# hsinnan75/Dart

Measured on AMD Instinct MI355X. Metric: M paired-end reads/sec (2x101 bp vs GRCh38-sized index), host to host; records bit-identical to CPU dart, higher is better.
Workload: dtype u64/u8 integer

## Files before the change

dart_amd/csrc/dg_pair.h:

```cpp
#pragma once
#include "../../include/dartgpu.h"
#include "dg_common.h"
#include "dg_chain.h"
#include "dg_report.h"

template <class R1, class R2>
__host__ __device__ inline void d_settle_pair(const DParams &pr, DRead &m1, R1 &p1, DRead &m2, R2 &p2)
{
    bool linked = p1.mate(m1.iBest) == m2.iBest;
    if (linked && !pr.multi_hit) return;
    if (!linked && m1.score > 0 && m2.score > 0) {
        int best_sum = 0;
        for (int i = 0; i < m1.CanNum; i++) {
            const int a = p1.aln(i), j = p1.mate(i);
            if (a <= 0 || j < 0) continue;
            const int b = p2.aln(j);
            if (b <= 0) continue;
            linked = true;
            if (a + b > best_sum) { best_sum = a + b; m1.iBest = i; m1.score = a; m2.iBest = j; m2.score = b; }
        }
    }
    if (linked) {
        for (int i = 0; i < m1.CanNum; i++) {
            const int j = p1.mate(i);
// ... 129 lines not shown
    for (int i = 1; i < n; i++) {
        const SKey x = key[i * S];
        int j = i;
        for (; j > 0 && key[(j - 1) * S] > x; j--) key[j * S] = key[(j - 1) * S];
        key[j * S] = x;
    }
}

#define SMALL_NW 8
__host__ __device__ inline bool d_small_nw_is_diagonal(uint64_t a8, uint64_t b8, int g)
{
    int sp[SMALL_NW], tp[SMALL_NW];
    uint8_t cb[SMALL_NW];
#pragma unroll
    for (int q = 0; q < SMALL_NW; q++) { sp[q] = -2 - (q + 1); tp[q] = -131072; cb[q] = q < g ? d_nt4((unsigned char)(b8 >> (8 * q))) : (uint8_t)7; }
    int diag0 = 0;
    bool leaves = false;
    for (int i = 1; i <= g; i++) {
        int left_s = -2 - i, left_r = -131072;
        const uint8_t ca = d_nt4((unsigned char)(a8 >> (8 * (i - 1))));
        int diag = diag0;
        diag0 = left_s;
#pragma unroll
        for (int q = 0; q < SMALL_NW; q++) {
            int x = left_r - 1, y = left_s - 3;
            const int r = x > y ? x : y;
            x = tp[q] - 1; y = sp[q] - 3;
            const int t = x > y ? x : y;
            const int sv = d_tr2(d_max3(diag + (ca == cb[q] ? 3 : -3), r, t));
            leaves = leaves || (q == i - 1 && (sv == r || sv == t));
            diag = sp[q];
            sp[q] = sv; tp[q] = t;
            left_s = sv; left_r = r;
        }
    }
    return !leaves;
}

struct ReadAscii {
    const unsigned char *p;
    __host__ __device__ __forceinline__ uint64_t get8(int i, int e) const { uint64_t v = 0; for (int t = 0; t < e; t++) v |= (uint64_t)p[i + t] << (8 * t); return v; }
    __host__ __device__ __forceinline__ int mismatches8(const DIndex &ix, int i, int e, int64_t g, bool &dash) const {
        const uint64_t ref = d_ref8(ix, g), a8 = get8(i, e), keep = e == 8 ? ~0ull : (1ull << (8 * e)) - 1ull, lo7 = 0x7F7F7F7F7F7F7F7Full, hi1 = 0x8080808080808080ull;
        const uint64_t x = (a8 ^ ref) & keep, y = (a8 ^ 0x2D2D2D2D2D2D2D2Dull) | ~keep;
        dash = dash || ((~(((y & lo7) + lo7) | y)) & hi1) != 0ull;
        return __builtin_popcountll((((x & lo7) + lo7) | x) & hi1);
    }
};
struct ReadWords {
    const uint32_t *w; int W2;
    __host__ __device__ __forceinline__ uint64_t get8(int i, int e) const {
        const int w0 = i >> 4, sh = (i & 15) << 1;
        const uint32_t chi = w[w0], clo = w0 + 1 < W2 ? w[w0 + 1] : 0u, mhi = w[W2 + w0], mlo = w0 + 1 < W2 ? w[W2 + w0 + 1] : 0xFFFFFFFFu;
        const uint32_t c16 = (sh ? (chi << sh) | (clo >> (32 - sh)) : chi) >> 16, m16 = (sh ? (mhi << sh) | (mlo >> (32 - sh)) : mhi) >> 16;
        uint64_t v = 0;
        for (int t = 0; t < e; t++) {
            const uint32_t c = (c16 >> (14 - 2 * t)) & 3u, m = (m16 >> (14 - 2 * t)) & 3u;
            v |= (uint64_t)(m ? 0x4Eu : ((0x54474341u >> (8u * c)) & 0xFFu)) << (8 * t);
        }
        return v;
    }
    __host__ __device__ __forceinline__ int mismatches8(const DIndex &ix, int i, int e, int64_t g, bool &dash) const {
        const int64_t L = ix.l_pac;
        uint32_t g16;
        if (g >= 0 && g + 8 <= L) g16 = (__builtin_bswap32(*(const uint32_a1 *)(ix.pac + (g >> 2))) << ((g & 3) << 1)) >> 16;
        else if (g >= L && g + 8 <= 2 * L) {
            const int64_t lo = 2 * L - 1 - g - 7;
            const uint32_t w = (__builtin_bswap32(*(const uint32_a1 *)(ix.pac + (lo >> 2))) << ((lo & 3) << 1)) >> 16;
            uint32_t r = ((w & 0x3333u) << 2) | ((w >> 2) & 0x3333u); r = ((r & 0x0F0Fu) << 4) | ((r >> 4) & 0x0F0Fu); r = ((r & 0x00FFu) << 8) | (r >> 8);
            g16 = ~r & 0xFFFFu;
        } else {
            const uint64_t ref = d_ref8(ix, g), a8 = get8(i, e), keep = e == 8 ? ~0ull : (1ull << (8 * e)) - 1ull, lo7 = 0x7F7F7F7F7F7F7F7Full, hi1 = 0x8080808080808080ull;
            const uint64_t x = (a8 ^ ref) & keep;
            return __builtin_popcountll((((x & lo7) + lo7) | x) & hi1);
        }
        const int w0 = i >> 4, sh = (i & 15) << 1;
        const uint32_t chi = w[w0], clo = w0 + 1 < W2 ? w[w0 + 1] : 0u, mhi = w[W2 + w0], mlo = w0 + 1 < W2 ? w[W2 + w0 + 1] : 0xFFFFFFFFu;
        const uint32_t c16 = (sh ? (chi << sh) | (clo >> (32 - sh)) : chi) >> 16, m16 = (sh ? (mhi << sh) | (mlo >> (32 - sh)) : mhi) >> 16;
        const uint32_t x = c16 ^ g16, keep = (0xFFFF0000u >> (2 * e)) & 0xFFFFu;
        return __builtin_popcount(((x | (x >> 1)) | m16) & 0x5555u & keep);
    }
};

template <int S, class RD>
__host__ __device__ inline bool d_unit_reports(const DIndex &ix, const LocTab &lt, const DParams &pr, bool first, const RD seq, int len,
                                               const SKey *key, uint32_t *cw, int nc, uint64_t *rw, int &n_slot, DRead &rd, uint32_t &n_cig, uint32_t &n_nw, uint32_t &n_cells)
{
    const int64_t L = ix.l_pac;
    rd.score = rd.sub_score = rd.mis_num = rd.mapq = rd.iBest = 0;
    rd.CanNum = nc > 0 ? nc : 1;
    for (int i = 0; i < nc; i++) {
        const uint32_t w = cw[i * S];
        if (cw_score(w) == 0) continue;
        const int n = cw_count(w), f = cw_first(w);
        const SKey k0 = key[f * S];
        const int64_t diag = sk_diag(k0);
        if (n > 1 && diag == -1) return false;
        SKey prev = k0;
        int aln = sk_rlen(k0), mis = 0;
        uint32_t calls = 0, cells = 0;
        for (int k = 1; k < n; k++) {
            const SKey cur = key[(f + k) * S];
            const int from = sk_rpos(prev) + sk_rlen(prev), g = sk_rpos(cur) - from;
            if (sk_diag(cur) != diag || g < 1) return false;
            const int64_t gp = sk_gpos(prev) + sk_rlen(prev);
            int nm = 0;
            bool dash = false;
            for (int q = 0; q < g; q += 8) nm += seq.mismatches8(ix, from + q, g - q < 8 ? g - q : 8, gp + q, dash);
            if (nm <= 2 && nm <= (int)(g * 0.2)) { aln += g - nm; mis += nm; }
            else if (g == 1 && !dash) { calls++; cells++; mis += 1; }
            else if (g <= SMALL_NW && !dash && d_small_nw_is_diagonal(seq.get8(from, g), d_ref8(ix, gp), g)) {
                calls++; cells += (uint32_t)(g * g); aln += g - nm; mis += nm;
            }
            else return false;
            aln += sk_rlen(cur);
            prev = cur;
        }
        const int64_t gPos = sk_gpos(k0), end_gPos = sk_gpos(prev) + sk_rlen(prev) - 1;
        if (n > 1 && ((gPos < L) != (end_gPos < L))) return false;
        const int head = sk_rpos(k0), span = sk_rpos(prev) + sk_rlen(prev) - head, tail = len - head - span;
        if (mis > pr.max_mismatch) aln = 0;
        if (n_slot >= PU_SLOTS) return false;
        const int slot = n_slot++;
        uint64_t w0 = 0;
        if (aln > 0) {
            const int lb = d_loc_lower_bound(lt, gPos);
            const int chr = lt.chr[lb];
            int64_t pos; int bdir;
            if (gPos < L) { bdir = first ? 1 : 0; pos = gPos + 1 - lt.off[chr]; }
            else { bdir = first ? 0 : 1; pos = lt.key[lb] - end_gPos + 1; }
            if (pos <= 0 || pos > 0xFFFFFFFFll || chr > 0xFFFF) return false;
            w0 = (uint64_t)pos | ((uint64_t)chr << 32) | ((uint64_t)aln << 48) | ((uint64_t)bdir << 60) | (1ull << 61);
            n_cig += 1u + (head > 0) + (tail > 0);
            if (aln > rd.score) { rd.iBest = i; rd.mis_num = mis; rd.sub_score = rd.score; rd.score = aln; }
            else if (aln == rd.score) rd.sub_score = rd.score;
        }
        rw[(2 * slot) * S] = w0;
        rw[(2 * slot + 1) * S] = (uint64_t)head | ((uint64_t)span << 12) | ((uint64_t)tail << 24) | ((uint64_t)mis << 48);
        cw[i * S] = (w & ~(15u << 27)) | ((uint32_t)slot << 27);
        n_nw += calls; n_cells += cells;
    }
    return true;
}

template <int S, class RD>
__host__ __device__ inline void d_unit_process_rd(const DIndex &ix, const LocTab &lt, const DParams &pr, bool paired, int n1, int n2, int len1, int len2,
                                               const RD seq1, const RD seq2, SKey *key, uint32_t *cw, uint64_t *rw,
                                               bool try_fast, UnitState &st)
{
    d_unit_sort<S>(key, n1);
    if (paired) d_unit_sort<S>(key + n1 * S, n2);
    int k = 0;
    st.nc[0] = d_cluster_seeds(lt, pr, len1, n1, [&](int i) { return key[i * S]; },
                               [&](int first, int count, int score, int64_t) { cw[(k++) * S] = cw_make(first, count, score); });
    st.nc[1] = 0;
    CandLds<S> a{key, cw, st.nc[0]}, b{key + n1 * S, cw + st.nc[0] * S, 0};
    if (paired) {
        st.nc[1] = b.cnt = d_cluster_seeds(lt, pr, len2, n2, [&](int i) { return key[(n1 + i) * S]; },
                                           [&](int first, int count, int score, int64_t) { cw[(k++) * S] = cw_make(first, count, score); });
    }
    PP_STAMP(st.pp, st.pt, 1);
    d_candidate_rules(paired, a, b);
    PP_STAMP(st.pp, st.pt, 2);
    st.fast = false; st.n_cig = 0; st.n_nw = st.n_cells = 0; st.flag0[0] = st.flag0[1] = 0;
    if (!try_fast) return;
    int n_slot = 0;
    uint32_t n_cig = 0, n_nw = 0, n_cells = 0;
    if (!d_unit_reports<S>(ix, lt, pr, true, seq1, len1, key, cw, st.nc[0], rw, n_slot, st.rd[0], n_cig, n_nw, n_cells)) return;
    if (paired && !d_unit_reports<S>(ix, lt, pr, false, seq2, len2, key + n1 * S, cw + st.nc[0] * S, st.nc[1], rw, n_slot, st.rd[1], n_cig, n_nw, n_cells)) return;
    PP_STAMP(st.pp, st.pt, 3);
    RepLds<S> p1{cw, rw, st.nc[0], 0}, p2{cw + st.nc[0] * S, rw, st.nc[1], 0};
    if (paired) {
        d_settle_pair(pr, st.rd[0], p1, st.rd[1], p2);
        d_flag_pair(st.rd[0], p1, st.rd[1], p2);
        d_mapq(st.rd[1], p2);
    } else d_flag_single(st.rd[0], p1);
    d_mapq(st.rd[0], p1);
    st.flag0[0] = p1.flag0; st.flag0[1] = p2.flag0;
    st.fast = true; st.n_cig = n_cig; st.n_nw = n_nw; st.n_cells = n_cells;
    PP_STAMP(st.pp, st.pt, 4);
}
template <int S>
__host__ __device__ inline void d_unit_process(const DIndex &ix, const DParams &pr, bool paired, int n1, int n2, int len1, int len2,
                                               const unsigned char *seq1, const unsigned char *seq2, SKey *key, uint32_t *cw, uint64_t *rw,
                                               bool try_fast, UnitState &st)
{
    d_unit_process_rd<S, ReadAscii>(ix, d_loc_tab(ix), pr, paired, n1, n2, len1, len2, ReadAscii{seq1}, ReadAscii{seq2}, key, cw, rw, try_fast, st);
}

struct CompactOut { dg_read_c *reads; dg_report_c *reports; uint32_t *cigar; unsigned int *bad; };
__host__ __device__ __forceinline__ bool d_compact_read(const dg_read_out &r, dg_read_c &o)
{
    o.score = (uint16_t)r.score; o.sub_score = (uint16_t)r.sub_score; o.mis_num = (uint16_t)r.mis_num; o.mapq = (uint8_t)r.mapq; o.n_sj = (uint8_t)r.n_sj;
    o.n_rep = (uint16_t)r.n_rep; o.best = (uint16_t)r.best;
    return !((uint32_t)r.score > 0xFFFFu || (uint32_t)r.sub_score > 0xFFFFu || (uint32_t)r.mis_num > 0xFFFFu || (uint32_t)r.mapq > 0xFFu || (uint32_t)r.n_sj > 0xFFu ||
             (uint32_t)r.n_rep > 0xFFFFu || (uint32_t)r.best > 0xFFFFu);
}
__host__ __device__ __forceinline__ bool d_compact_report(const dg_report_out &p, bool plain, bool slow, dg_report_c &q)
{
    q.pos = (int32_t)p.pos; q.aln_score = (uint16_t)p.aln_score; q.flag = (uint16_t)p.flag; q.paired_idx = (int16_t)p.paired_idx;
    q.chr = p.chr < 0 ? (uint16_t)0xFFFFu : (uint16_t)p.chr; q.sj_type = (int8_t)p.sj_type; q.bdir = (uint8_t)p.bdir; q.pad = slow ? 1u : 0u;
    q.n_cigar = plain ? (uint8_t)DG_CIGAR_FULL_MATCH : (uint8_t)p.n_cigar;
    return !(p.pos != (int64_t)(int32_t)p.pos || (uint32_t)p.aln_score > 0xFFFFu || (uint32_t)p.flag > 0xFFFFu || p.paired_idx > 32767 || p.paired_idx < -1 ||
             p.chr >= 0xFFFF || p.n_cigar > 254u || p.sj_type < -128 || p.sj_type > 127 || (uint32_t)p.bdir > 1u);
}

template <int S>
__host__ __device__ inline uint32_t d_unit_compact_ops(const DRead &rd, const RepLds<S> &p)
{
    uint32_t n = 0;
    for (int i = 0; i < rd.CanNum; i++) {
        const int s = p.slot(i);
        if (s == 15) continue;
        const uint64_t w0 = p.rw[(2 * s) * S], w1 = p.rw[(2 * s + 1) * S];
        if (!((w0 >> 61) & 1ull)) continue;
        const uint32_t head = (uint32_t)(w1 & 0xFFFu), tail = (uint32_t)((w1 >> 24) & 0xFFFu);
        n += (head || tail) ? 1u + (head > 0) + (tail > 0) : 0u;
    }
    return n;
}

template <int S>
__host__ __device__ inline uint32_t d_unit_emit_read(bool first, const DRead &rd, const RepLds<S> &p, uint32_t rep_off, uint32_t cig_off,
                                                     dg_read_out *rout_r, dg_report_out *reports, uint32_t *cigar, const CompactOut &co = CompactOut{nullptr, nullptr, nullptr, nullptr},
                                                     dg_read_c *rc_r = nullptr, uint32_t cigc_off = 0, bool full = true)
{
    dg_read_out o;
    o.score = rd.score; o.sub_score = rd.sub_score; o.mis_num = rd.mis_num; o.mapq = rd.mapq; o.n_rep = rd.CanNum; o.best = rd.iBest;
    o.rep_off = (int32_t)rep_off; o.sj_off = 0; o.n_sj = 0;
    if (full) *rout_r = o;
    bool fits = true;
    if (co.reads) { dg_read_c oc; fits = d_compact_read(o, oc); *rc_r = oc; }
    uint32_t used = 0, used_c = 0;
    for (int i = 0; i < rd.CanNum; i++) {
        dg_report_out rp;
        rp.aln_score = 0; rp.sj_type = -1; rp.flag = p.flag(i); rp.paired_idx = p.mate(i); rp.chr = -1; rp.bdir = 0; rp.pos = 0;
        rp.cigar_off = cig_off + used; rp.n_cigar = 0;
        const int s = p.slot(i);
        if (s != 15) {
            const uint64_t w0 = p.rw[(2 * s) * S], w1 = p.rw[(2 * s + 1) * S];
            if ((w0 >> 61) & 1ull) {
                rp.aln_score = (int32_t)((w0 >> 48) & 0xFFFu); rp.chr = (int32_t)((w0 >> 32) & 0xFFFFu); rp.bdir = (int32_t)((w0 >> 60) & 1u);
                rp.pos = (int64_t)(w0 & 0xFFFFFFFFull);
                const uint32_t head = (uint32_t)(w1 & 0xFFFu), span = (uint32_t)((w1 >> 12) & 0xFFFu), tail = (uint32_t)((w1 >> 24) & 0xFFFu);
                const bool rev = (rp.bdir != 0) != first;
                const uint32_t lead = rev ? tail : head, trail = rev ? head : tail;
                const uint32_t o_mid = CIG(span, OP_M), o_trail = CIG(trail, OP_S);
                const uint32_t a0 = lead ? CIG(lead, OP_S) : o_mid, a1 = lead ? o_mid : o_trail, a2 = o_trail;
                const uint32_t m = 1u + (lead ? 1u : 0u) + (trail ? 1u : 0u);
                if (full) { uint32_t *c = cigar + cig_off + used; c[0] = a0; if (m > 1) c[1] = a1; if (m > 2) c[2] = a2; }
                rp.n_cigar = m; used += m;
                if (co.reads && m > 1) { uint32_t *c = co.cigar + cigc_off + used_c; c[0] = a0; c[1] = a1; if (m > 2) c[2] = a2; used_c += m; }
            }
        }
        if (full) reports[rep_off + (uint32_t)i] = rp;
        if (co.reads) { dg_report_c q; fits = d_compact_report(rp, rp.n_cigar == 1u, false, q) && fits; co.reports[rep_off + (uint32_t)i] = q; }
    }
    if (co.reads && !fits) *co.bad = 1u;
    return used;
}

#include "dg_scan.h"

__device__ __forceinline__ uint32_t d_pac_touch(const DIndex &ix, SKey k)
{
    const int64_t L = ix.l_pac, g = sk_gpos(k) + sk_rlen(k);
    if (g >= 0 && g + 8 <= L) return *(const uint32_a1 *)(ix.pac + (g >> 2));
    if (g >= L && g + 8 <= 2 * L) return *(const uint32_a1 *)(ix.pac + ((2 * L - 1 - g - 7) >> 2));
    return 0u;
}

template <bool PACKED>
__global__ void __launch_bounds__(PU_THREADS)
k_pair(const DIndex ix, const DParams pr, int n_units, int paired, int try_fast, int write_all_sorted ,
       const unsigned char *__restrict__ seq, const uint32_t *__restrict__ seq_off, const uint32_t *__restrict__ enc, int W2, const uint16_t *__restrict__ rlen,
       const uint32_t *__restrict__ seed_off, SKey *__restrict__ seeds, DCand *__restrict__ cands, uint32_t *__restrict__ ncand,
       uint32_t *__restrict__ rep_off, uint32_t *__restrict__ slow_units,
       dg_read_out *__restrict__ rout, dg_report_out *__restrict__ reports, uint32_t *__restrict__ cigar,
       uint32_t cap_rep, uint32_t cap_cig, TileScan ts, DSizes *sizes, unsigned int *pool_top, unsigned long long *ctr, int *err, const CompactOut co)
{
    const unsigned long long t_wave0 = wall_clock64();
    __shared__ SKey s_key[PU_SEEDS * PU_THREADS];
    __shared__ uint32_t s_cw[PU_SEEDS * PU_THREADS];
    __shared__ uint64_t s_rw[2 * PU_SLOTS * PU_THREADS];
    __shared__ unsigned long long s_scan[20];
    __shared__ unsigned int s_tile;
    __shared__ int64_t s_lkey[PU_LOC_MAX]; __shared__ int64_t s_coff[PU_LOC_MAX / 2]; __shared__ int32_t s_lchr[PU_LOC_MAX];
    const bool tab_in_lds = 2 * ix.n_chr <= PU_LOC_MAX;
    if (tab_in_lds) {
        for (int i = threadIdx.x; i < 2 * ix.n_chr; i += PU_THREADS) { s_lkey[i] = ix.loc_key[i]; s_lchr[i] = ix.loc_chr[i]; }
        for (int i = threadIdx.x; i < ix.n_chr; i += PU_THREADS) s_coff[i] = ix.chr_off[i];
    }
    const LocTab lt = tab_in_lds ? LocTab{s_lkey, s_lchr, s_coff, 2 * ix.n_chr} : d_loc_tab(ix);
    bool leave = false;
    if (threadIdx.x == 0) { const int e0 = __hip_atomic_load(err, __ATOMIC_RELAXED, __HIP_MEMORY_SCOPE_AGENT); leave = e0 == DG_E_SEEDS || e0 == DG_E_SEEDQ || e0 == DG_E_SCAN; }
    const unsigned int tile = d_tile_ticket_unless(ts, &s_tile, leave);
    if (tile == SCAN_LEAVE) return;
    const int u = (int)(tile * PU_THREADS + threadIdx.x);
    const bool valid = u < n_units;
    SKey *key = s_key + threadIdx.x;
    uint32_t *cw = s_cw + threadIdx.x;
    uint64_t *rw = s_rw + threadIdx.x;
    UnitState st;
    st.fast = false; st.n_cig = 0; st.n_nw = st.n_cells = 0; st.nc[0] = st.nc[1] = 0; st.flag0[0] = st.flag0[1] = 0;
#ifdef DG_PAIR_PROF
    for (int i = 0; i < 10; i++) st.pp[i] = 0;
    st.pt = __builtin_amdgcn_s_memtime();
    const unsigned long long pp_t0 = st.pt;
#endif
    int r1 = 0, n1 = 0, n2 = 0, len1 = 0, len2 = 0;
    uint32_t b1 = 0;
    uint32_t pf = 0, pf2 = 0, pf3 = 0, pf4 = 0, pf5 = 0, pf6 = 0;
    bool heavy = false;
    if (valid) {
        r1 = paired ? 2 * u : u;
        len1 = rlen[r1]; len2 = paired ? rlen[r1 + 1] : 0;
        if (PACKED) { pf = enc[(size_t)r1 * 2 * W2 + (W2 >> 1)]; if (paired) pf2 = enc[(size_t)(r1 + 1) * 2 * W2 + (W2 >> 1)]; }
        b1 = seed_off[r1];
        const uint32_t e1 = seed_off[r1 + 1], e2 = paired ? seed_off[r1 + 2] : e1;
        n1 = (int)(e1 - b1); n2 = (int)(e2 - e1);
        heavy = n1 + n2 > PU_SEEDS;
        if (!heavy) {
            const SKey *src = seeds + b1;
            const int nt = n1 + n2;
            for (int i0 = 0; i0 < nt; i0 += 4) {
                const SKey k0 = src[i0], k1 = i0 + 1 < nt ? src[i0 + 1] : 0, k2 = i0 + 2 < nt ? src[i0 + 2] : 0, k3 = i0 + 3 < nt ? src[i0 + 3] : 0;
                key[i0 * PU_THREADS] = k0;
                if (i0 + 1 < nt) key[(i0 + 1) * PU_THREADS] = k1;
                if (i0 + 2 < nt) key[(i0 + 2) * PU_THREADS] = k2;
                if (i0 + 3 < nt) key[(i0 + 3) * PU_THREADS] = k3;
            }
#ifdef __HIP_DEVICE_COMPILE__
            __asm__ volatile("" ::: "memory");
#endif
            if (n1 > 1) { pf3 = d_pac_touch(ix, key[0]); if (n1 > 2) pf4 = d_pac_touch(ix, key[1 * PU_THREADS]); }
            if (n2 > 1) { pf5 = d_pac_touch(ix, key[n1 * PU_THREADS]); if (n2 > 2) pf6 = d_pac_touch(ix, key[(n1 + 1) * PU_THREADS]); }
            PP_STAMP(st.pp, st.pt, 0);
            if (PACKED) {
                const ReadWords a{enc + (size_t)r1 * 2 * W2, W2}, b{enc + (size_t)(r1 + (paired ? 1 : 0)) * 2 * W2, W2};
                d_unit_process_rd<PU_THREADS, ReadWords>(ix, lt, pr, paired != 0, n1, n2, len1, len2, a, b, key, cw, rw, try_fast != 0, st);
            } else d_unit_process_rd<PU_THREADS, ReadAscii>(ix, lt, pr, paired != 0, n1, n2, len1, len2, ReadAscii{seq + seq_off[r1]}, ReadAscii{seq + seq_off[r1 + (paired ? 1 : 0)]}, key, cw, rw, try_fast != 0, st);
        } else { st.nc[0] = (int)ncand[r1]; st.nc[1] = paired ? (int)ncand[r1 + 1] : 0; }
    }
    const uint32_t nrep1 = valid ? (uint32_t)(st.nc[0] > 0 ? st.nc[0] : 1) : 0u, nrep2 = (valid && paired) ? (uint32_t)(st.nc[1] > 0 ? st.nc[1] : 1) : 0u;
    Triple mine, tot;
    mine.x = nrep1 + nrep2; mine.y = (valid && !st.fast) ? 1u : 0u; mine.z = st.fast ? st.n_cig : 0u;
    uint32_t cc1 = 0;
    mine.w = 0;
    if (co.reads && st.fast) {
        RepLds<PU_THREADS> q1{cw, rw, st.nc[0], st.flag0[0]}, q2{cw + st.nc[0] * PU_THREADS, rw, st.nc[1], st.flag0[1]};
        cc1 = d_unit_compact_ops<PU_THREADS>(st.rd[0], q1);
        mine.w = cc1 + (paired ? d_unit_compact_ops<PU_THREADS>(st.rd[1], q2) : 0u);
    }
    PP_STAMP(st.pp, st.pt, 5);
    const Triple inb = d_block_exclusive(mine, tot, s_scan);
    PP_STAMP(st.pp, st.pt, 6);
    const Triple base = d_tile_exclusive(ts, tile, tot, s_scan + 16, err);
    PP_STAMP(st.pp, st.pt, 7);
    const uint32_t rep0 = base.x + inb.x, slow_at = base.y + inb.y;
    const uint64_t cig0 = base.z + inb.z;
    unsigned long long n_cands = 0, n_nw = 0, n_cells = 0;
    if (valid) {
        rep_off[r1] = rep0;
        if (paired) rep_off[r1 + 1] = rep0 + nrep1;
        if (!heavy) n_cands = (unsigned long long)(st.nc[0] + st.nc[1]);
        if (st.fast) {
            if ((uint64_t)rep0 + mine.x > cap_rep) atomicMax(err, DG_E_REPORTS);
            else if (cig0 + st.n_cig > cap_cig) atomicMax(err, DG_E_CIGFINAL);
            else {
                RepLds<PU_THREADS> p1{cw, rw, st.nc[0], st.flag0[0]}, p2{cw + st.nc[0] * PU_THREADS, rw, st.nc[1], st.flag0[1]};
                const uint32_t cigc0 = base.w + inb.w;
                const bool full = !(write_all_sorted & 2) || !co.reads;
                const uint32_t c1 = d_unit_emit_read<PU_THREADS>(true, st.rd[0], p1, rep0, (uint32_t)cig0, rout + r1, reports, cigar, co, co.reads ? co.reads + r1 : nullptr, cigc0, full);
                if (paired) d_unit_emit_read<PU_THREADS>(false, st.rd[1], p2, rep0 + nrep1, (uint32_t)cig0 + c1, rout + r1 + 1, reports, cigar, co, co.reads ? co.reads + r1 + 1 : nullptr, cigc0 + cc1, full);
                n_nw = st.n_nw; n_cells = st.n_cells;
            }
        } else {
            if (slow_at < (uint32_t)n_units) slow_units[slow_at] = (uint32_t)u;
            if ((uint64_t)rep0 + mine.x > cap_rep) atomicMax(err, DG_E_REPORTS);
        }
        if (!heavy && (!st.fast || (write_all_sorted & 1))) {
            const int nt = n1 + n2;
            for (int i = 0; i < nt; i++) seeds[b1 + i] = key[i * PU_THREADS];
            auto put_cands = [&](int first_cw, int first_key, uint32_t seg, int count, int r) {
                for (int i = 0; i < count; i++) {
                    const uint32_t w = cw[(first_cw + i) * PU_THREADS];
                    const int64_t d = sk_diag(key[(first_key + cw_first(w)) * PU_THREADS]);
                    DCand c = d_new_cand(seg + (uint32_t)cw_first(w), cw_count(w), cw_score(w), d < 0 ? 0 : d);
                    c.PairedIdx = cw_mate(w);
                    cands[seg + i] = c;
                }
                ncand[r] = (uint32_t)count;
            };
            put_cands(0, 0, b1, st.nc[0], r1);
            if (paired) put_cands(st.nc[0], n1, b1 + (uint32_t)n1, st.nc[1], r1 + 1);
        } else if (!heavy) { ncand[r1] = (uint32_t)st.nc[0]; if (paired) ncand[r1 + 1] = (uint32_t)st.nc[1]; }
    }
    if (tile == gridDim.x - 1 && threadIdx.x == 0) {
        sizes->total_rep = base.x + tot.x; sizes->n_slow_units = base.y + tot.y; sizes->cig_fast = (uint32_t)(base.z + tot.z);
        sizes->total_cig = sizes->cig_fast;
        sizes->pad[2] = base.w + tot.w;
        *pool_top = (base.x + tot.x) * CIG_SLOT;
    }
    PP_STAMP(st.pp, st.pt, 8);
#ifdef DG_PAIR_PROF
    if ((threadIdx.x & 63) == 0 && (tile % 61u) == 0u)
        printf("kpair tile %u wave %d: total %llu | load %llu sort+cluster %llu rules %llu reports %llu settle %llu rest %llu blockscan %llu lookback %llu emit %llu\n", tile, (int)(threadIdx.x >> 6),
               __builtin_amdgcn_s_memtime() - pp_t0, st.pp[0], st.pp[1], st.pp[2], st.pp[3], st.pp[4], st.pp[5], st.pp[6], st.pp[7], st.pp[8]);
#endif
    if (n_units < 0 && (pf ^ pf2 ^ pf3 ^ pf4 ^ pf5 ^ pf6) == 0x5A17C3E1u) atomicMax(err, DG_E_SCAN);
    d_wave_add(ctr + CTR_CANDS, n_cands);
    d_wave_add(ctr + CTR_NW, n_nw);
    d_wave_add(ctr + CTR_NWCELLS, n_cells);
    d_wave_resident(ctr, CTR_WT_PAIR, t_wave0);
}
```

Baseline: 1173.

## Distribute per-candidate report building and emission across wave lanes

Splits per-read report construction into independent per-candidate work items. Each lane handles its first candidate locally, and the remaining candidates are redistributed across the wave through a prefix scan and an owner search. Report emission and seed/candidate write-out are redistributed in the same way, so one lane no longer serialises all of its candidates. The goal is to reduce lane divergence and load imbalance from reads with many candidates. The cost is extra shuffles, wave-level LDS synchronisation, and calls/cells counters packed into the report word.

Result: no change. 1165 (-0.7%).

```diff
diff --git a/dart_amd/csrc/dg_pair.h b/dart_amd/csrc/dg_pair.h
--- a/dart_amd/csrc/dg_pair.h
+++ b/dart_amd/csrc/dg_pair.h
@@ -235,71 +235,96 @@
     }
 };
 
+#define PU_OUTSIDE (~0ull)
+#define PU_W1_SPENT ((0xFull << 60) | (0xFFFull << 36))
 template <int S, class RD>
-__host__ __device__ inline bool d_unit_reports(const DIndex &ix, const LocTab &lt, const DParams &pr, bool first, const RD seq, int len,
-                                               const SKey *key, uint32_t *cw, int nc, uint64_t *rw, int &n_slot, DRead &rd, uint32_t &n_cig, uint32_t &n_nw, uint32_t &n_cells)
+__host__ __device__ inline bool d_cand_report(const DIndex &ix, const LocTab &lt, const DParams &pr, bool first, const RD seq, int len,
+                                              const SKey *key, uint32_t w, uint64_t *rw, int slot)
 {
     const int64_t L = ix.l_pac;
+    rw[(2 * slot + 1) * S] = PU_OUTSIDE;
+    const int n = cw_count(w), f = cw_first(w);
+    const SKey k0 = key[f * S];
+    const int64_t diag = sk_diag(k0);
+    if (n > 1 && diag == -1) return false;
+    SKey prev = k0;
+    int aln = sk_rlen(k0), mis = 0;
+    uint32_t calls = 0, cells = 0;
+    for (int k = 1; k < n; k++) {
+        const SKey cur = key[(f + k) * S];
+        const int from = sk_rpos(prev) + sk_rlen(prev), g = sk_rpos(cur) - from;
+        if (sk_diag(cur) != diag || g < 1) return false;
+        const int64_t gp = sk_gpos(prev) + sk_rlen(prev);
+        int nm = 0;
+        bool dash = false;
+        for (int q = 0; q < g; q += 8) nm += seq.mismatches8(ix, from + q, g - q < 8 ? g - q : 8, gp + q, dash);
+        if (nm <= 2 && nm <= (int)(g * 0.2)) { aln += g - nm; mis += nm; }
+        else if (g == 1 && !dash) { calls++; cells++; mis += 1; }
+        else if (g <= SMALL_NW && !dash && d_small_nw_is_diagonal(seq.get8(from, g), d_ref8(ix, gp), g)) {
+            calls++; cells += (uint32_t)(g * g); aln += g - nm; mis += nm;
+        }
+        else return false;
+        aln += sk_rlen(cur);
+        prev = cur;
+    }
+    const int64_t gPos = sk_gpos(k0), end_gPos = sk_gpos(prev) + sk_rlen(prev) - 1;
+    if (n > 1 && ((gPos < L) != (end_gPos < L))) return false;
+    const int head = sk_rpos(k0), span = sk_rpos(prev) + sk_rlen(prev) - head, tail = len - head - span;
+    if (mis > pr.max_mismatch) aln = 0;
+    uint64_t w0 = 0;
+    if (aln > 0) {
+        const int lb = d_loc_lower_bound(lt, gPos);
+        const int chr = lt.chr[lb];
+        int64_t pos; int bdir;
+        if (gPos < L) { bdir = first ? 1 : 0; pos = gPos + 1 - lt.off[chr]; }
+        else { bdir = first ? 0 : 1; pos = lt.key[lb] - end_gPos + 1; }
+        if (pos <= 0 || pos > 0xFFFFFFFFll || chr > 0xFFFF) return false;
+        w0 = (uint64_t)pos | ((uint64_t)chr << 32) | ((uint64_t)aln << 48) | ((uint64_t)bdir << 60) | (1ull << 61);
+    }
+    if (calls > 15u || cells > 0xFFFu) return false;
+    rw[(2 * slot) * S] = w0;
+    rw[(2 * slot + 1) * S] = (uint64_t)head | ((uint64_t)span << 12) | ((uint64_t)tail << 24) | ((uint64_t)mis << 48) | ((uint64_t)cells << 36) | ((uint64_t)calls << 60);
+    return true;
+}
+
+template <int S>
+__host__ __device__ inline uint32_t d_unit_slots(uint32_t *cw, int nc)
+{
+    uint32_t live = 0, k = 0;
+    for (int i = 0; i < nc; i++) {
+        const uint32_t w = cw[i * S];
+        if (cw_score(w) == 0) continue;
+        cw[i * S] = (w & ~(15u << 27)) | ((k < 15u ? k : 15u) << 27);
+        live |= 1u << i; k++;
+    }
+    return live;
+}
+
+template <int S>
+__host__ __device__ inline bool d_mate_replay(const uint32_t *cw, int nc, uint64_t *rw, DRead &rd, uint32_t &n_cig, uint32_t &n_nw, uint32_t &n_cells)
+{
     rd.score = rd.sub_score = rd.mis_num = rd.mapq = rd.iBest = 0;
     rd.CanNum = nc > 0 ? nc : 1;
     for (int i = 0; i < nc; i++) {
         const uint32_t w = cw[i * S];
         if (cw_score(w) == 0) continue;
-        const int n = cw_count(w), f = cw_first(w);
-        const SKey k0 = key[f * S];
-        const int64_t diag = sk_diag(k0);
-        if (n > 1 && diag == -1) return false;
-        SKey prev = k0;
-        int aln = sk_rlen(k0), mis = 0;
-        uint32_t calls = 0, cells = 0;
-        for (int k = 1; k < n; k++) {
-            const SKey cur = key[(f + k) * S];
-            const int from = sk_rpos(prev) + sk_rlen(prev), g = sk_rpos(cur) - from;
-            if (sk_diag(cur) != diag || g < 1) return false;
-            const int64_t gp = sk_gpos(prev) + sk_rlen(prev);
-            int nm = 0;
-            bool dash = false;
-            for (int q = 0; q < g; q += 8) nm += seq.mismatches8(ix, from + q, g - q < 8 ? g - q : 8, gp + q, dash);
-            if (nm <= 2 && nm <= (int)(g * 0.2)) { aln += g - nm; mis += nm; }
-            else if (g == 1 && !dash) { calls++; cells++; mis += 1; }
-            else if (g <= SMALL_NW && !dash && d_small_nw_is_diagonal(seq.get8(from, g), d_ref8(ix, gp), g)) {
-                calls++; cells += (uint32_t)(g * g); aln += g - nm; mis += nm;
-            }
-            else return false;
-            aln += sk_rlen(cur);
-            prev = cur;
-        }
-        const int64_t gPos = sk_gpos(k0), end_gPos = sk_gpos(prev) + sk_rlen(prev) - 1;
-        if (n > 1 && ((gPos < L) != (end_gPos < L))) return false;
-        const int head = sk_rpos(k0), span = sk_rpos(prev) + sk_rlen(prev) - head, tail = len - head - span;
-        if (mis > pr.max_mismatch) aln = 0;
-        if (n_slot >= PU_SLOTS) return false;
-        const int slot = n_slot++;
-        uint64_t w0 = 0;
+        const int slot = cw_slot(w);
+        const uint64_t w0 = rw[(2 * slot) * S], w1 = rw[(2 * slot + 1) * S];
+        if (w1 == PU_OUTSIDE) return false;
+        n_nw += (uint32_t)(w1 >> 60); n_cells += (uint32_t)((w1 >> 36) & 0xFFFu);
+        rw[(2 * slot + 1) * S] = w1 & ~PU_W1_SPENT;
+        const int aln = (int)((w0 >> 48) & 0xFFFu);
         if (aln > 0) {
-            const int lb = d_loc_lower_bound(lt, gPos);
-            const int chr = lt.chr[lb];
-            int64_t pos; int bdir;
-            if (gPos < L) { bdir = first ? 1 : 0; pos = gPos + 1 - lt.off[chr]; }
-            else { bdir = first ? 0 : 1; pos = lt.key[lb] - end_gPos + 1; }
-            if (pos <= 0 || pos > 0xFFFFFFFFll || chr > 0xFFFF) return false;
-            w0 = (uint64_t)pos | ((uint64_t)chr << 32) | ((uint64_t)aln << 48) | ((uint64_t)bdir << 60) | (1ull << 61);
-            n_cig += 1u + (head > 0) + (tail > 0);
-            if (aln > rd.score) { rd.iBest = i; rd.mis_num = mis; rd.sub_score = rd.score; rd.score = aln; }
+            n_cig += 1u + ((w1 & 0xFFFu) != 0) + (((w1 >> 24) & 0xFFFu) != 0);
+            if (aln > rd.score) { rd.iBest = i; rd.mis_num = (int)((w1 >> 48) & 0xFFFu); rd.sub_score = rd.score; rd.score = aln; }
             else if (aln == rd.score) rd.sub_score = rd.score;
         }
-        rw[(2 * slot) * S] = w0;
-        rw[(2 * slot + 1) * S] = (uint64_t)head | ((uint64_t)span << 12) | ((uint64_t)tail << 24) | ((uint64_t)mis << 48);
-        cw[i * S] = (w & ~(15u << 27)) | ((uint32_t)slot << 27);
-        n_nw += calls; n_cells += cells;
     }
     return true;
 }
 
-template <int S, class RD>
-__host__ __device__ inline void d_unit_process_rd(const DIndex &ix, const LocTab &lt, const DParams &pr, bool paired, int n1, int n2, int len1, int len2,
-                                               const RD seq1, const RD seq2, SKey *key, uint32_t *cw, uint64_t *rw,
-                                               bool try_fast, UnitState &st)
+template <int S>
+__host__ __device__ inline void d_unit_candidates(const LocTab &lt, const DParams &pr, bool paired, int n1, int n2, int len1, int len2, SKey *key, uint32_t *cw, UnitState &st)
 {
     d_unit_sort<S>(key, n1);
     if (paired) d_unit_sort<S>(key + n1 * S, n2);
@@ -316,11 +341,14 @@
     d_candidate_rules(paired, a, b);
     PP_STAMP(st.pp, st.pt, 2);
     st.fast = false; st.n_cig = 0; st.n_nw = st.n_cells = 0; st.flag0[0] = st.flag0[1] = 0;
-    if (!try_fast) return;
-    int n_slot = 0;
+}
+
+template <int S>
+__host__ __device__ inline void d_unit_finish(const DParams &pr, bool paired, uint32_t *cw, uint64_t *rw, UnitState &st)
+{
     uint32_t n_cig = 0, n_nw = 0, n_cells = 0;
-    if (!d_unit_reports<S>(ix, lt, pr, true, seq1, len1, key, cw, st.nc[0], rw, n_slot, st.rd[0], n_cig, n_nw, n_cells)) return;
-    if (paired && !d_unit_reports<S>(ix, lt, pr, false, seq2, len2, key + n1 * S, cw + st.nc[0] * S, st.nc[1], rw, n_slot, st.rd[1], n_cig, n_nw, n_cells)) return;
+    if (!d_mate_replay<S>(cw, st.nc[0], rw, st.rd[0], n_cig, n_nw, n_cells)) return;
+    if (paired && !d_mate_replay<S>(cw + st.nc[0] * S, st.nc[1], rw, st.rd[1], n_cig, n_nw, n_cells)) return;
     PP_STAMP(st.pp, st.pt, 3);
     RepLds<S> p1{cw, rw, st.nc[0], 0}, p2{cw + st.nc[0] * S, rw, st.nc[1], 0};
     if (paired) {
@@ -333,6 +361,25 @@
     st.fast = true; st.n_cig = n_cig; st.n_nw = n_nw; st.n_cells = n_cells;
     PP_STAMP(st.pp, st.pt, 4);
 }
+
+template <int S, class RD>
+__host__ __device__ inline void d_unit_process_rd(const DIndex &ix, const LocTab &lt, const DParams &pr, bool paired, int n1, int n2, int len1, int len2,
+                                               const RD seq1, const RD seq2, SKey *key, uint32_t *cw, uint64_t *rw,
+                                               bool try_fast, UnitState &st)
+{
+    d_unit_candidates<S>(lt, pr, paired, n1, n2, len1, len2, key, cw, st);
+    if (!try_fast) return;
+    const uint32_t live = d_unit_slots<S>(cw, st.nc[0] + st.nc[1]);
+    if (__builtin_popcount(live) > PU_SLOTS) return;
+    for (int i = 0; i < st.nc[0] + st.nc[1]; i++) {
+        if (!((live >> i) & 1u)) continue;
+        const uint32_t w = cw[i * S];
+        const bool second = i >= st.nc[0];
+        if (!(second ? d_cand_report<S, RD>(ix, lt, pr, false, seq2, len2, key + n1 * S, w, rw, cw_slot(w))
+                     : d_cand_report<S, RD>(ix, lt, pr, true, seq1, len1, key, w, rw, cw_slot(w)))) return;
+    }
+    d_unit_finish<S>(pr, paired, cw, rw, st);
+}
 template <int S>
 __host__ __device__ inline void d_unit_process(const DIndex &ix, const DParams &pr, bool paired, int n1, int n2, int len1, int len2,
                                                const unsigned char *seq1, const unsigned char *seq2, SKey *key, uint32_t *cw, uint64_t *rw,
@@ -359,24 +406,60 @@
 }
 
 template <int S>
-__host__ __device__ inline uint32_t d_unit_compact_ops(const DRead &rd, const RepLds<S> &p)
+__host__ __device__ __forceinline__ uint32_t d_report_ops(const RepLds<S> &p, int i)
+{
+    const int s = p.slot(i);
+    if (s == 15) return 0u;
+    const uint64_t w0 = p.rw[(2 * s) * S], w1 = p.rw[(2 * s + 1) * S];
+    if (!((w0 >> 61) & 1ull)) return 0u;
+    const uint32_t head = (uint32_t)(w1 & 0xFFFu), tail = (uint32_t)((w1 >> 24) & 0xFFFu);
+    const uint32_t m = 1u + (head > 0) + (tail > 0);
+    return m | ((m > 1u ? m : 0u) << 16);
+}
+template <int S>
+__host__ __device__ inline uint32_t d_unit_ops(const DRead &rd, const RepLds<S> &p)
 {
     uint32_t n = 0;
-    for (int i = 0; i < rd.CanNum; i++) {
-        const int s = p.slot(i);
-        if (s == 15) continue;
+    for (int i = 0; i < rd.CanNum; i++) n += d_report_ops<S>(p, i);
+    return n;
+}
+template <int S>
+__host__ __device__ inline uint32_t d_unit_compact_ops(const DRead &rd, const RepLds<S> &p) { return d_unit_ops<S>(rd, p) >> 16; }
+
+template <int S>
+__host__ __device__ __forceinline__ uint32_t d_emit_report(bool first, const RepLds<S> &p, int i, uint32_t rep_at, uint32_t cig_at, uint32_t cigc_at,
+                                                           dg_report_out *reports, uint32_t *cigar, const CompactOut &co, bool full, bool &fits, uint32_t &ops_c)
+{
+    dg_report_out rp;
+    rp.aln_score = 0; rp.sj_type = -1; rp.flag = p.flag(i); rp.paired_idx = p.mate(i); rp.chr = -1; rp.bdir = 0; rp.pos = 0;
+    rp.cigar_off = cig_at; rp.n_cigar = 0;
+    ops_c = 0;
+    const int s = p.slot(i);
+    if (s != 15) {
         const uint64_t w0 = p.rw[(2 * s) * S], w1 = p.rw[(2 * s + 1) * S];
-        if (!((w0 >> 61) & 1ull)) continue;
-        const uint32_t head = (uint32_t)(w1 & 0xFFFu), tail = (uint32_t)((w1 >> 24) & 0xFFFu);
-        n += (head || tail) ? 1u + (head > 0) + (tail > 0) : 0u;
-    }
-    return n;
+        if ((w0 >> 61) & 1ull) {
+            rp.aln_score = (int32_t)((w0 >> 48) & 0xFFFu); rp.chr = (int32_t)((w0 >> 32) & 0xFFFFu); rp.bdir = (int32_t)((w0 >> 60) & 1u);
+            rp.pos = (int64_t)(w0 & 0xFFFFFFFFull);
+            const uint32_t head = (uint32_t)(w1 & 0xFFFu), span = (uint32_t)((w1 >> 12) & 0xFFFu), tail = (uint32_t)((w1 >> 24) & 0xFFFu);
+            const bool rev = (rp.bdir != 0) != first;
+            const uint32_t lead = rev ? tail : head, trail = rev ? head : tail;
+            const uint32_t o_mid = CIG(span, OP_M), o_trail = CIG(trail, OP_S);
+            const uint32_t a0 = lead ? CIG(lead, OP_S) : o_mid, a1 = lead ? o_mid : o_trail, a2 = o_trail;
+            const uint32_t m = 1u + (lead ? 1u : 0u) + (trail ? 1u : 0u);
+            if (full) { uint32_t *c = cigar + cig_at; c[0] = a0; if (m > 1) c[1] = a1; if (m > 2) c[2] = a2; }
+            rp.n_cigar = m;
+            if (co.reads && m > 1) { uint32_t *c = co.cigar + cigc_at; c[0] = a0; c[1] = a1; if (m > 2) c[2] = a2; ops_c = m; }
+        }
+    }
+    if (full) reports[rep_at] = rp;
+    if (co.reads) { dg_report_c q; fits = d_compact_report(rp, rp.n_cigar == 1u, false, q) && fits; co.reports[rep_at] = q; }
+    return rp.n_cigar;
 }
 
 template <int S>
 __host__ __device__ inline uint32_t d_unit_emit_read(bool first, const DRead &rd, const RepLds<S> &p, uint32_t rep_off, uint32_t cig_off,
                                                      dg_read_out *rout_r, dg_report_out *reports, uint32_t *cigar, const CompactOut &co = CompactOut{nullptr, nullptr, nullptr, nullptr},
-                                                     dg_read_c *rc_r = nullptr, uint32_t cigc_off = 0, bool full = true)
+                                                     dg_read_c *rc_r = nullptr, uint32_t cigc_off = 0, bool full = true, bool only_first = false)
 {
     dg_read_out o;
     o.score = rd.score; o.sub_score = rd.sub_score; o.mis_num = rd.mis_num; o.mapq = rd.mapq; o.n_rep = rd.CanNum; o.best = rd.iBest;
@@ -385,32 +468,78 @@
     bool fits = true;
     if (co.reads) { dg_read_c oc; fits = d_compact_read(o, oc); *rc_r = oc; }
     uint32_t used = 0, used_c = 0;
-    for (int i = 0; i < rd.CanNum; i++) {
-        dg_report_out rp;
-        rp.aln_score = 0; rp.sj_type = -1; rp.flag = p.flag(i); rp.paired_idx = p.mate(i); rp.chr = -1; rp.bdir = 0; rp.pos = 0;
-        rp.cigar_off = cig_off + used; rp.n_cigar = 0;
-        const int s = p.slot(i);
-        if (s != 15) {
-            const uint64_t w0 = p.rw[(2 * s) * S], w1 = p.rw[(2 * s + 1) * S];
-            if ((w0 >> 61) & 1ull) {
-                rp.aln_score = (int32_t)((w0 >> 48) & 0xFFFu); rp.chr = (int32_t)((w0 >> 32) & 0xFFFFu); rp.bdir = (int32_t)((w0 >> 60) & 1u);
-                rp.pos = (int64_t)(w0 & 0xFFFFFFFFull);
-                const uint32_t head = (uint32_t)(w1 & 0xFFFu), span = (uint32_t)((w1 >> 12) & 0xFFFu), tail = (uint32_t)((w1 >> 24) & 0xFFFu);
-                const bool rev = (rp.bdir != 0) != first;
-                const uint32_t lead = rev ? tail : head, trail = rev ? head : tail;
-                const uint32_t o_mid = CIG(span, OP_M), o_trail = CIG(trail, OP_S);
-                const uint32_t a0 = lead ? CIG(lead, OP_S) : o_mid, a1 = lead ? o_mid : o_trail, a2 = o_trail;
-                const uint32_t m = 1u + (lead ? 1u : 0u) + (trail ? 1u : 0u);
-                if (full) { uint32_t *c = cigar + cig_off + used; c[0] = a0; if (m > 1) c[1] = a1; if (m > 2) c[2] = a2; }
-                rp.n_cigar = m; used += m;
-                if (co.reads && m > 1) { uint32_t *c = co.cigar + cigc_off + used_c; c[0] = a0; c[1] = a1; if (m > 2) c[2] = a2; used_c += m; }
-            }
-        }
-        if (full) reports[rep_off + (uint32_t)i] = rp;
-        if (co.reads) { dg_report_c q; fits = d_compact_report(rp, rp.n_cigar == 1u, false, q) && fits; co.reports[rep_off + (uint32_t)i] = q; }
+    const int n = only_first ? 1 : rd.CanNum;
+    for (int i = 0; i < n; i++) {
+        uint32_t ops_c;
+        used += d_emit_report<S>(first, p, i, rep_off + (uint32_t)i, cig_off + used, cigc_off + used_c, reports, cigar, co, full, fits, ops_c);
+        used_c += ops_c;
     }
     if (co.reads && !fits) *co.bad = 1u;
     return used;
+}
+
+__device__ __forceinline__ void d_wave_lds_sync()
+{
+#ifdef __HIP_DEVICE_COMPILE__
+    __builtin_amdgcn_fence(__ATOMIC_RELEASE, "wavefront");
+    __builtin_amdgcn_wave_barrier();
+    __builtin_amdgcn_fence(__ATOMIC_ACQUIRE, "wavefront");
+#endif
+}
+__device__ __forceinline__ uint32_t d_wave_inclusive(uint32_t v)
+{
+    const int lane = (int)(threadIdx.x & 63u);
+    for (int o = 1; o < 64; o <<= 1) { const uint32_t up = (uint32_t)__shfl_up((int)v, o, 64); if (lane >= o) v += up; }
+    return v;
+}
+__device__ __forceinline__ int d_wave_owner(uint32_t incl, uint32_t j)
+{
+    int own = 0;
+    for (int step = 32; step; step >>= 1) { const uint32_t v = (uint32_t)__shfl((int)incl, own + step - 1, 64); if (v <= j) own += step; }
+    return own & 63;
+}
+
+template <int S>
+__host__ __device__ inline void d_item_emit_report(bool first, const RepLds<S> &p, int i, uint32_t rep_first, uint32_t cig_first, uint32_t cigc_first,
+                                                   dg_report_out *reports, uint32_t *cigar, const CompactOut &co, bool full)
+{
+    uint32_t before = 0;
+    for (int j = 0; j < i; j++) before += d_report_ops<S>(p, j);
+    bool fits = true;
+    uint32_t ops_c;
+    d_emit_report<S>(first, p, i, rep_first + (uint32_t)i, cig_first + (before & 0xFFFFu), cigc_first + (before >> 16), reports, cigar, co, full, fits, ops_c);
+    if (co.reads && !fits) *co.bad = 1u;
+}
+__host__ __device__ __forceinline__ int pu_extra_reports(int nc) { return nc > 1 ? nc - 1 : 0; }
+__host__ __device__ __forceinline__ void pu_item_report(int nc0, int k, int &mate, int &i)
+{
+    const int e0 = pu_extra_reports(nc0);
+    mate = k >= e0 ? 1 : 0;
+    i = (mate ? k - e0 : k) + 1;
+}
+__device__ __forceinline__ void d_wave_emit_reports(bool emit, int nc0, int nc1, uint32_t rep0, uint32_t cig0, uint32_t cigc0, uint32_t ops1, uint32_t *s_cw, uint64_t *s_rw,
+                                                    dg_report_out *reports, uint32_t *cigar, const CompactOut &co, bool full)
+{
+    const int lane = (int)(threadIdx.x & 63u), wave0 = (int)(threadIdx.x & ~63u);
+    uint32_t incl = emit ? (uint32_t)(pu_extra_reports(nc0) + pu_extra_reports(nc1)) : 0u;
+    if (__ballot(incl != 0u) == 0ull) return;
+    incl = d_wave_inclusive(incl);
+    const uint32_t total = (uint32_t)__shfl((int)incl, 63, 64), pk = (uint32_t)nc0 | ((uint32_t)nc1 << 5);
+    for (uint32_t base = 0; base < total; base += 64u) {
+        const uint32_t j = base + (uint32_t)lane;
+        const int own = d_wave_owner(incl, j);
+        const uint32_t o_incl = (uint32_t)__shfl((int)incl, own, 64), o_pk = (uint32_t)__shfl((int)pk, own, 64), o_rep0 = (uint32_t)__shfl((int)rep0, own, 64),
+                       o_cig0 = (uint32_t)__shfl((int)cig0, own, 64), o_cigc0 = (uint32_t)__shfl((int)cigc0, own, 64), o_ops1 = (uint32_t)__shfl((int)ops1, own, 64);
+        if (j < total) {
+            const int c0 = (int)(o_pk & 31u), c1 = (int)(o_pk >> 5);
+            int mate, i;
+            pu_item_report(c0, (int)(j - (o_incl - (uint32_t)(pu_extra_reports(c0) + pu_extra_reports(c1)))), mate, i);
+            const int t = wave0 + own;
+            const RepLds<PU_THREADS> p{s_cw + t + (mate ? c0 * PU_THREADS : 0), s_rw + t, mate ? c1 : c0, 0};
+            d_item_emit_report<PU_THREADS>(mate == 0, p, i, o_rep0 + (mate ? (uint32_t)(c0 > 0 ? c0 : 1) : 0u), o_cig0 + (mate ? (o_ops1 & 0xFFFFu) : 0u), o_cigc0 + (mate ? (o_ops1 >> 16) : 0u),
+                                           reports, cigar, co, full);
+        }
+    }
 }
 
 #include "dg_scan.h"
@@ -421,6 +550,100 @@
     if (g >= 0 && g + 8 <= L) return *(const uint32_a1 *)(ix.pac + (g >> 2));
     if (g >= L && g + 8 <= 2 * L) return *(const uint32_a1 *)(ix.pac + ((2 * L - 1 - g - 7) >> 2));
     return 0u;
+}
+
+template <int S>
+__host__ __device__ __forceinline__ void d_item_put_cand(const SKey *key, const uint32_t *cw, int n1, int nc0, uint32_t b1, int i, DCand *__restrict__ cands)
+{
+    const bool second = i >= nc0;
+    const int first_key = second ? n1 : 0;
+    const uint32_t seg = b1 + (uint32_t)first_key, w = cw[i * S];
+    const int64_t d = sk_diag(key[(first_key + cw_first(w)) * S]);
+    DCand c = d_new_cand(seg + (uint32_t)cw_first(w), cw_count(w), cw_score(w), d < 0 ? 0 : d);
+    c.PairedIdx = cw_mate(w);
+    cands[seg + (uint32_t)(i - (second ? nc0 : 0))] = c;
+}
+#define PU_ITEM_GROUP 16
+__host__ __device__ __forceinline__ uint32_t pu_counts_pack(int n1, int n2, int nc0, int nc1) { return (uint32_t)n1 | ((uint32_t)n2 << 5) | ((uint32_t)nc0 << 10) | ((uint32_t)nc1 << 15); }
+template <int S>
+__host__ __device__ __forceinline__ void d_item_write_out(const SKey *key, const uint32_t *cw, uint32_t pk, uint32_t b1, int i, SKey *__restrict__ seeds, DCand *__restrict__ cands)
+{
+    const int n1 = (int)(pk & 31u), n2 = (int)((pk >> 5) & 31u), nc0 = (int)((pk >> 10) & 31u), nc1 = (int)((pk >> 15) & 31u);
+    if (i < n1 + n2) seeds[b1 + (uint32_t)i] = key[i * S];
+    if (i < nc0 + nc1) d_item_put_cand<S>(key, cw, n1, nc0, b1, i, cands);
+}
+__host__ __device__ __forceinline__ int pu_take_owner(unsigned long long &m)
+{
+    const int o = m ? (int)__builtin_ctzll(m) : -1;
+    m &= m - 1ull;
+    return o;
+}
+static_assert(PU_ITEM_GROUP == PU_SEEDS && 64 / PU_ITEM_GROUP == 4 && PU_SEEDS < 32, "a group of lanes covers a unit's seeds, four groups a wave; the counts fit five bits");
+__device__ __forceinline__ void d_wave_write_out(bool wr, uint32_t pk, uint32_t b1, const SKey *s_key, const uint32_t *s_cw, SKey *__restrict__ seeds, DCand *__restrict__ cands)
+{
+    unsigned long long m = __ballot(wr);
+    const int lane = (int)(threadIdx.x & 63u), wave0 = (int)(threadIdx.x & ~63u), grp = lane / PU_ITEM_GROUP, i = lane % PU_ITEM_GROUP;
+    while (m) {
+        const int o0 = pu_take_owner(m), o1 = pu_take_owner(m), o2 = pu_take_owner(m), o3 = pu_take_owner(m);
+        const int o = grp == 0 ? o0 : (grp == 1 ? o1 : (grp == 2 ? o2 : o3));
+        const uint32_t opk = (uint32_t)__shfl((int)pk, o < 0 ? lane : o, 64), ob1 = (uint32_t)__shfl((int)b1, o < 0 ? lane : o, 64);
+        if (o >= 0) d_item_write_out<PU_THREADS>(s_key + wave0 + o, s_cw + wave0 + o, opk, ob1, i, seeds, cands);
+    }
+}
+
+__host__ __device__ __forceinline__ uint32_t pu_report_items(uint32_t live, int nc0) { return live & ~1u & ~(1u << nc0); }
+__host__ __device__ __forceinline__ int pu_kth_bit(uint32_t x, int k) { for (int t = 0; t < k; t++) x &= x - 1u; return __builtin_ctz(x); }
+template <bool PACKED> struct PuRead;
+template <> struct PuRead<true> {
+    __device__ static __forceinline__ ReadWords of(const unsigned char *, const uint32_t *, const uint32_t *enc, int W2, int r) { return ReadWords{enc + (size_t)r * 2 * W2, W2}; }
+};
+template <> struct PuRead<false> {
+    __device__ static __forceinline__ ReadAscii of(const unsigned char *seq, const uint32_t *seq_off, const uint32_t *, int, int r) { return ReadAscii{seq + seq_off[r]}; }
+};
+template <bool PACKED>
+__device__ __forceinline__ void d_wave_reports(const DIndex &ix, const LocTab &lt, const DParams &pr, bool go, int paired, int u, int n1, int len1, int len2,
+                                               const unsigned char *seq, const uint32_t *seq_off, const uint32_t *enc, int W2, const uint16_t *rlen,
+                                               SKey *s_key, uint32_t *s_cw, uint64_t *s_rw, UnitState &st)
+{
+    typedef PuRead<PACKED> R;
+    const int lane = (int)(threadIdx.x & 63u), wave0 = (int)(threadIdx.x & ~63u);
+    SKey *key = s_key + threadIdx.x; uint32_t *cw = s_cw + threadIdx.x; uint64_t *rw = s_rw + threadIdx.x;
+    const int r1 = paired ? 2 * u : u;
+    uint32_t live = 0;
+    bool ok = false;
+    if (go) {
+        live = d_unit_slots<PU_THREADS>(cw, st.nc[0] + st.nc[1]);
+        ok = __builtin_popcount(live) <= PU_SLOTS;
+#pragma unroll 1
+        for (int m = 0; m < 2; m++) {
+            const int c = m ? st.nc[0] : 0;
+            if (!ok || !((live >> c) & 1u)) continue;
+            const uint32_t w = cw[c * PU_THREADS];
+            ok = d_cand_report<PU_THREADS>(ix, lt, pr, m == 0, R::of(seq, seq_off, enc, W2, r1 + m), m ? len2 : len1, key + (m ? n1 * PU_THREADS : 0), w, rw, cw_slot(w));
+        }
+    }
+    const uint32_t items = ok ? pu_report_items(live, st.nc[0]) : 0u;
+    if (__ballot(items != 0u) != 0ull) {
+        const uint32_t incl = d_wave_inclusive((uint32_t)__builtin_popcount(items)), total = (uint32_t)__shfl((int)incl, 63, 64);
+        const uint32_t pk = live | ((uint32_t)n1 << 16) | ((uint32_t)st.nc[0] << 21);
+        d_wave_lds_sync();
+        for (uint32_t base = 0; base < total; base += 64u) {
+            const uint32_t j = base + (uint32_t)lane;
+            const int own = d_wave_owner(incl, j);
+            const uint32_t o_incl = (uint32_t)__shfl((int)incl, own, 64), o_pk = (uint32_t)__shfl((int)pk, own, 64);
+            if (j < total) {
+                const int o_n1 = (int)((o_pk >> 16) & 31u), o_nc0 = (int)((o_pk >> 21) & 31u);
+                const uint32_t o_items = pu_report_items(o_pk & 0xFFFFu, o_nc0);
+                const int c = pu_kth_bit(o_items, (int)(j - (o_incl - (uint32_t)__builtin_popcount(o_items))));
+                const bool second = c >= o_nc0;
+                const int ot = wave0 + own, ou = u - lane + own, r = (paired ? 2 * ou : ou) + (second ? 1 : 0);
+                const uint32_t w = s_cw[ot + c * PU_THREADS];
+                d_cand_report<PU_THREADS>(ix, lt, pr, !second, R::of(seq, seq_off, enc, W2, r), (int)rlen[r], s_key + ot + (second ? o_n1 * PU_THREADS : 0), w, s_rw + ot, cw_slot(w));
+            }
+        }
+        d_wave_lds_sync();
+    }
+    if (ok) d_unit_finish<PU_THREADS>(pr, paired != 0, cw, rw, st);
 }
 
 template <bool PACKED>
@@ -489,21 +712,20 @@
             if (n1 > 1) { pf3 = d_pac_touch(ix, key[0]); if (n1 > 2) pf4 = d_pac_touch(ix, key[1 * PU_THREADS]); }
             if (n2 > 1) { pf5 = d_pac_touch(ix, key[n1 * PU_THREADS]); if (n2 > 2) pf6 = d_pac_touch(ix, key[(n1 + 1) * PU_THREADS]); }
             PP_STAMP(st.pp, st.pt, 0);
-            if (PACKED) {
-                const ReadWords a{enc + (size_t)r1 * 2 * W2, W2}, b{enc + (size_t)(r1 + (paired ? 1 : 0)) * 2 * W2, W2};
-                d_unit_process_rd<PU_THREADS, ReadWords>(ix, lt, pr, paired != 0, n1, n2, len1, len2, a, b, key, cw, rw, try_fast != 0, st);
-            } else d_unit_process_rd<PU_THREADS, ReadAscii>(ix, lt, pr, paired != 0, n1, n2, len1, len2, ReadAscii{seq + seq_off[r1]}, ReadAscii{seq + seq_off[r1 + (paired ? 1 : 0)]}, key, cw, rw, try_fast != 0, st);
+            d_unit_candidates<PU_THREADS>(lt, pr, paired != 0, n1, n2, len1, len2, key, cw, st);
         } else { st.nc[0] = (int)ncand[r1]; st.nc[1] = paired ? (int)ncand[r1 + 1] : 0; }
     }
+    d_wave_reports<PACKED>(ix, lt, pr, valid && !heavy && try_fast != 0, paired, u, n1, len1, len2, seq, seq_off, enc, W2, rlen, s_key, s_cw, s_rw, st);
     const uint32_t nrep1 = valid ? (uint32_t)(st.nc[0] > 0 ? st.nc[0] : 1) : 0u, nrep2 = (valid && paired) ? (uint32_t)(st.nc[1] > 0 ? st.nc[1] : 1) : 0u;
     Triple mine, tot;
     mine.x = nrep1 + nrep2; mine.y = (valid && !st.fast) ? 1u : 0u; mine.z = st.fast ? st.n_cig : 0u;
     uint32_t cc1 = 0;
     mine.w = 0;
-    if (co.reads && st.fast) {
+    uint32_t ops1 = 0;
+    if (st.fast) {
         RepLds<PU_THREADS> q1{cw, rw, st.nc[0], st.flag0[0]}, q2{cw + st.nc[0] * PU_THREADS, rw, st.nc[1], st.flag0[1]};
-        cc1 = d_unit_compact_ops<PU_THREADS>(st.rd[0], q1);
-        mine.w = cc1 + (paired ? d_unit_compact_ops<PU_THREADS>(st.rd[1], q2) : 0u);
+        ops1 = d_unit_ops<PU_THREADS>(st.rd[0], q1);
+        if (co.reads) { cc1 = ops1 >> 16; mine.w = cc1 + (paired ? d_unit_compact_ops<PU_THREADS>(st.rd[1], q2) : 0u); }
     }
     PP_STAMP(st.pp, st.pt, 5);
     const Triple inb = d_block_exclusive(mine, tot, s_scan);
@@ -513,6 +735,9 @@
     const uint32_t rep0 = base.x + inb.x, slow_at = base.y + inb.y;
     const uint64_t cig0 = base.z + inb.z;
     unsigned long long n_cands = 0, n_nw = 0, n_cells = 0;
+    const uint32_t cigc0 = base.w + inb.w;
+    const bool full = !(write_all_sorted & 2) || !co.reads;
+    bool emit = false;
     if (valid) {
         rep_off[r1] = rep0;
         if (paired) rep_off[r1 + 1] = rep0 + nrep1;
@@ -522,33 +747,19 @@
             else if (cig0 + st.n_cig > cap_cig) atomicMax(err, DG_E_CIGFINAL);
             else {
                 RepLds<PU_THREADS> p1{cw, rw, st.nc[0], st.flag0[0]}, p2{cw + st.nc[0] * PU_THREADS, rw, st.nc[1], st.flag0[1]};
-                const uint32_t cigc0 = base.w + inb.w;
-                const bool full = !(write_all_sorted & 2) || !co.reads;
-                const uint32_t c1 = d_unit_emit_read<PU_THREADS>(true, st.rd[0], p1, rep0, (uint32_t)cig0, rout + r1, reports, cigar, co, co.reads ? co.reads + r1 : nullptr, cigc0, full);
-                if (paired) d_unit_emit_read<PU_THREADS>(false, st.rd[1], p2, rep0 + nrep1, (uint32_t)cig0 + c1, rout + r1 + 1, reports, cigar, co, co.reads ? co.reads + r1 + 1 : nullptr, cigc0 + cc1, full);
+                emit = true;
+                d_unit_emit_read<PU_THREADS>(true, st.rd[0], p1, rep0, (uint32_t)cig0, rout + r1, reports, cigar, co, co.reads ? co.reads + r1 : nullptr, cigc0, full, true);
+                if (paired) d_unit_emit_read<PU_THREADS>(false, st.rd[1], p2, rep0 + nrep1, (uint32_t)cig0 + (ops1 & 0xFFFFu), rout + r1 + 1, reports, cigar, co, co.reads ? co.reads + r1 + 1 : nullptr, cigc0 + cc1, full, true);
                 n_nw = st.n_nw; n_cells = st.n_cells;
             }
         } else {
             if (slow_at < (uint32_t)n_units) slow_units[slow_at] = (uint32_t)u;
             if ((uint64_t)rep0 + mine.x > cap_rep) atomicMax(err, DG_E_REPORTS);
         }
-        if (!heavy && (!st.fast || (write_all_sorted & 1))) {
-            const int nt = n1 + n2;
-            for (int i = 0; i < nt; i++) seeds[b1 + i] = key[i * PU_THREADS];
-            auto put_cands = [&](int first_cw, int first_key, uint32_t seg, int count, int r) {
-                for (int i = 0; i < count; i++) {
-                    const uint32_t w = cw[(first_cw + i) * PU_THREADS];
-                    const int64_t d = sk_diag(key[(first_key + cw_first(w)) * PU_THREADS]);
-                    DCand c = d_new_cand(seg + (uint32_t)cw_first(w), cw_count(w), cw_score(w), d < 0 ? 0 : d);
-                    c.PairedIdx = cw_mate(w);
-                    cands[seg + i] = c;
-                }
-                ncand[r] = (uint32_t)count;
-            };
-            put_cands(0, 0, b1, st.nc[0], r1);
-            if (paired) put_cands(st.nc[0], n1, b1 + (uint32_t)n1, st.nc[1], r1 + 1);
-        } else if (!heavy) { ncand[r1] = (uint32_t)st.nc[0]; if (paired) ncand[r1 + 1] = (uint32_t)st.nc[1]; }
-    }
+        if (!heavy) { ncand[r1] = (uint32_t)st.nc[0]; if (paired) ncand[r1 + 1] = (uint32_t)st.nc[1]; }
+    }
+    d_wave_emit_reports(emit, st.nc[0], st.nc[1], rep0, (uint32_t)cig0, cigc0, ops1, s_cw, s_rw, reports, cigar, co, full);
+    d_wave_write_out(valid && !heavy && (!st.fast || (write_all_sorted & 1)), pu_counts_pack(n1, n2, st.nc[0], st.nc[1]), b1, s_key, s_cw, seeds, cands);
     if (tile == gridDim.x - 1 && threadIdx.x == 0) {
         sizes->total_rep = base.x + tot.x; sizes->n_slow_units = base.y + tot.y; sizes->cig_fast = (uint32_t)(base.z + tot.z);
         sizes->total_cig = sizes->cig_fast;
```
